# wojciech-graj/C-Raytracer

Measured on AMD Instinct MI355X. Metric: Mrays/s (primary+secondary) at 1920×1080×64spp; 1/2/4/8 GPU, higher is better.
Workload: dtype f32

## Files before the change

c-raytracer_amd/csrc/rtx_ctx.cpp:

```cpp
#include <hip/hip_runtime.h>

#include <stdarg.h>
#include <stdio.h>
#include <string.h>

#include <algorithm>
#include <vector>

#include "rtx.h"
#include "rtx_device.h"
#include "rtx_kat.h"
#include "rtx_internal.h"

static thread_local char g_err[512] = "";

int rtx_fail(int code, const char *fmt, ...)
{
	va_list ap;
	va_start(ap, fmt);
	vsnprintf(g_err, sizeof(g_err), fmt, ap);
	va_end(ap);
	return code;
}

// ... 183 lines not shown
			return fail(RTX_ERR_ARG, "shadow point masks %lld is not 0 or 1", (long long)value);
		c->opt_point = (int)value;
		return RTX_OK;
	case RTX_OPT_SHADOW_DARK:
		if (value < 0 || value > 1)
			return fail(RTX_ERR_ARG, "shadow dark samples %lld is not 0 or 1", (long long)value);
		c->opt_dark = (int)value;
		return RTX_OK;
	case RTX_OPT_SHADOW_ORDER:
		if (value < 0 || value > 1)
			return fail(RTX_ERR_ARG, "shadow sample order %lld is not 0 or 1", (long long)value);
		c->opt_order = (int)value;
		return RTX_OK;
	case RTX_OPT_SHADOW_SPEC:
		if (value < 0 || value > 1)
			return fail(RTX_ERR_ARG, "shadow specular shortcut %lld is not 0 or 1", (long long)value);
		c->opt_spec = (int)value;
		return RTX_OK;
	case RTX_OPT_SHADOW_PREMASK:
		if (value < 0 || value > 1)
			return fail(RTX_ERR_ARG, "shadow pre-mask %lld is not 0 or 1", (long long)value);
		c->opt_premask = (int)value;
		return RTX_OK;
	}
	return fail(RTX_ERR_ARG, "unknown option %d", option);
}

extern "C" int rtx_read_wide_tree(rtx_ctx *c, void *entries, uint32_t capacity, uint32_t *count, float frame[6])
{
	if (!c || !count)
		return fail(RTX_ERR_ARG, "null argument");
	if (!c->have_scene)
		return fail(RTX_ERR_STATE, "rtx_read_wide_tree before rtx_upload_scene");
	const DScene &S = c->scene;
	*count = S.w8 ? S.num_w8 : 0u;
	if (frame) {
		memcpy(frame, S.w8qo, 12);
		memcpy(frame + 3, S.w8qs, 12);
	}
	if (entries && S.w8 && capacity) {
		HIP_TRY(hipSetDevice(c->device));
		HIP_TRY(hipMemcpy(entries, S.w8, (size_t)std::min(capacity, S.num_w8) * sizeof(DW8), hipMemcpyDeviceToHost));
	}
	return RTX_OK;
}

// ... 76 lines not shown
```

c-raytracer_amd/csrc/rtx_internal.h:

```cpp
#ifndef RTX_INTERNAL_H
#define RTX_INTERNAL_H

#include <hip/hip_runtime.h>

#include <algorithm>
#include <chrono>
#include <cstdio>
#include <cstring>
#include <vector>

#include "rtx.h"
#include "rtx_device.h"
#include "rtx_launch.h"

int rtx_fail(int code, const char *fmt, ...);
#define fail rtx_fail

#define HIP_TRY(expr)                                                                                   \
	do {                                                                                            \
		hipError_t e_ = (expr);                                                                 \
		if (e_ != hipSuccess)                                                                   \
			return fail(RTX_ERR_HIP, "%s failed: %s", #expr, hipGetErrorString(e_));        \
	} while (0)

// ... 57 lines not shown
	const int rc = upload(d.p, v, stream);
	if (!rc)
		d.bytes = std::max<size_t>(v.size(), 1) * sizeof(T);
	return rc;
}

#if RTX_MEASURE
struct PhaseClock {
	std::chrono::steady_clock::time_point t = std::chrono::steady_clock::now();
	void mark(const char *what, hipStream_t st)
	{
		(void)hipStreamSynchronize(st);
		const auto n = std::chrono::steady_clock::now();
		fprintf(stderr, "[rtx upload] %-24s %8.2f ms\n", what, std::chrono::duration<double, std::milli>(n - t).count());
		t = n;
	}
};
#define PHASE(clk, what, st) clk.mark(what, st)
#else
struct PhaseClock {};
#define PHASE(clk, what, st) ((void)clk)
#endif

struct SpKey {
	uint32_t v[21] = {};
	uint32_t set = 0;
	bool operator==(const SpKey &o) const { return set && o.set && std::equal(v, v + 21, o.v); }
};

struct RTX_HIDDEN CtxHandles {
	hipStream_t stream = nullptr;
	hipEvent_t ev0 = nullptr, ev1 = nullptr;
	hipEvent_t ev[5] = { nullptr, nullptr, nullptr, nullptr, nullptr };
	CtxHandles() = default;
	CtxHandles(const CtxHandles &) = delete;
	CtxHandles &operator=(const CtxHandles &) = delete;
	~CtxHandles()
	{
		for (hipEvent_t e : { ev[0], ev[1], ev[2], ev[3], ev[4], ev0, ev1 })
			if (e)
				(void)hipEventDestroy(e);
		if (stream)
			(void)hipStreamDestroy(stream);
	}
};

struct rtx_ctx : CtxHandles {
	RTX_HIDDEN ~rtx_ctx() = default;
	int device = 0;
	int builder = RTX_BUILD_SAH_GPU;
	int cus = 0;
	DNode *d_nodes = nullptr;
	DPlane *d_planes = nullptr;
	DMaterial *d_mats = nullptr;
	DEmitter *d_emitters = nullptr;
	DEmitter *d_lin = nullptr;
	DQNode *d_qnodes = nullptr;
	uint32_t *d_top = nullptr;
	DW8 *d_w8 = nullptr;
	DW8S *d_w8s = nullptr;
	float4 *d_cull = nullptr;
	float4 *d_lsph = nullptr;
	DScene scene{};
	bool have_scene = false;
	DevBuf<DTask> d_tasks;
	DevBuf<uint32_t> d_ostk;
	DevBuf<uint32_t> d_w8spill;
	DevBuf<float4> d_staging;
	DevBuf<float4> d_sp;
	DevBuf<float4> d_contrib;
	DevBuf<uint32_t> d_ordbuf;
	DevBuf<uint32_t> d_pmask;
	DevBuf<uint2> d_tile_rec;
	double sp_tile_seen = 0.0;
	SpKey sp_tile_key{};
	DevBuf<uint32_t> d_sortbuf;
	DevBuf<void> d_sorttmp;
	DevBuf<int> d_post_rad;
	DevBuf<float4> d_post_pv;
	DevBuf<unsigned> d_post_scratch;
	float bound_lo[3] = { 0, 0, 0 }, bound_hi[3] = { 0, 0, 0 };
	uint32_t total_lights = 0;
	DevBuf<unsigned long long> d_ctr;
	DevBuf<float> d_rgb, d_z;
	rtx_stats stats{};
	rtx_point_stats pstats{};
	rtx_dark_stats dstats{};
	rtx_order_stats ostats{};
// ... 19 lines not shown
	DevBuf<double> d_ad_vs;
	DevBuf<uint32_t> d_ad_tiles;
	DevBuf<float> d_ad_var;
	DevBuf<uint32_t> d_ad_passes;
	rtx_adaptive_stats ad_stats{};
	int opt_walk = RTX_WALK_AUTO;
	uint32_t opt_leaf = 1;
	bool opt_spsort = true;
	uint32_t opt_slot = 0;
	uint32_t opt_grab = 4096;
	uint32_t opt_lstk = RTX_W8_STACK;
	int opt_trace_walk = RTX_WALK_AUTO;
	int opt_frame = RTX_FRAME_AUTO;
	uint32_t opt_chunk = 0;
	uint32_t opt_sp_tile = 0;
	uint32_t opt_rays_grab = 0;
	uint32_t opt_rays_queues = 0;
	int opt_cull = 1;
	int opt_point = 1;
	int opt_dark = 1;
	int opt_spec = 1;
	int opt_order = 1;
	int opt_premask = 1;
	uint32_t mem_share = 1;
};

struct QFrame {
	float qo[3], qs[3];
};

struct HostScene {
	int builder = RTX_BUILD_SAH_HOST;
	int device = 0;
	bool recs_on_device = false;
	std::vector<DNode> recs;
	uint32_t nnodes = 0, nb = 0, root_ref = RTX_EMPTY_REF, depth = 0;
	std::vector<DQNode> qnodes;
	QFrame qf{};
	std::vector<uint32_t> qtop;
	uint32_t ntop = 0;
	std::vector<DW8> w8;
	std::vector<uint32_t> w8leaf;
	uint32_t w8depth = 0;
	QFrame w8f{};
	bool w8noemit = false;
	bool w8_on_device = false;
// ... 110 lines not shown
```

c-raytracer_amd/csrc/rtx_launch.h:

```cpp
#ifndef RTX_LAUNCH_H
#define RTX_LAUNCH_H

#include <hip/hip_runtime.h>

#include "rtx.h"

struct DNode;
struct DPrim;
struct DW8;
struct DW8S;
struct DMaterial;
struct DScene;
struct DFrame;
struct DParams;
struct DTask;

#define RTX_HIDDEN __attribute__((visibility("hidden")))

extern "C" {

hipError_t rtx_lbvh_build(uint32_t n, const float *d_lo, const float *d_hi, const DPrim *d_prims_in, const float blo[3],
			  const float bhi[3], uint32_t max_leaf, DNode **recs_out, uint32_t *nnodes_out, uint32_t *root_out,
			  uint32_t *depth_out, hipStream_t st);
hipError_t rtx_ploc_build(uint32_t n, const float *d_lo, const float *d_hi, const DPrim *d_prims_in, const float blo[3],
			  const float bhi[3], uint32_t max_leaf, DNode **recs_out, uint32_t *nnodes_out, uint32_t *root_out,
			  uint32_t *depth_out, uint32_t *rounds_out, hipStream_t st);
hipError_t rtx_sah_build(uint32_t n, const float *d_lo, const float *d_hi, const DPrim *d_prims_in, uint32_t max_leaf,
			 uint32_t bins, uint32_t max_depth, float c_trav, float c_isect, DNode **recs_out, uint32_t *nnodes_out,
			 uint32_t *root_out, uint32_t *depth_out, uint32_t *levels_out, hipStream_t st);
hipError_t rtx_launch_find_prims(const DPrim *prims, uint32_t n, const uint32_t *objs, uint32_t nobj, uint32_t *out,
				 hipStream_t stream);
RTX_HIDDEN hipError_t rtx_load_build(void);

hipError_t rtx_launch_w8_scalar(uint32_t n, const DW8 *w8, const uint32_t *leafmap, DW8S *w8s, hipStream_t st);
hipError_t rtx_w8_collapse_device(const DNode *recs, uint32_t nnodes, uint32_t nb, const uint32_t *skip_obj,
				  uint32_t num_objects, DW8 **w8_out, DW8S **w8s_out, uint32_t **leafmap_out,
				  uint32_t *entries_out, uint32_t *scalar_entries_out, uint32_t *depth_out, uint32_t *wide_out,
				  uint32_t *top_out, float qo[3], float qs[3], hipStream_t st);
RTX_HIDDEN hipError_t rtx_load_wide8_dev(void);

size_t rtx_trace_lds_bytes(uint32_t stack_size);
hipError_t rtx_trace_occupancy(uint32_t stack_size, int *blocks_per_cu);
hipError_t rtx_launch_trace(const DScene *S, const DFrame *F, const DParams *P, float *rgb, float *z, DTask *tasks,
			    uint32_t task_cap, float4 *staging, uint32_t staging_cap, float4 *sp_out, uint32_t sp_cap,
			    uint2 *tile_rec, uint32_t tile_begin, uint32_t tile_end, unsigned long long *ctr, uint32_t waves,
			    int count, const uint32_t *tile_list, hipStream_t stream);
hipError_t rtx_launch_accum(const DFrame *F, const DParams *P, const uint2 *tile_rec, const float4 *contrib,
			    uint32_t tile_begin, uint32_t ntiles, float *rgb, const uint32_t *tile_list, hipStream_t stream);
size_t rtx_rays_lds_bytes(uint32_t stack_size);
hipError_t rtx_rays_occupancy(uint32_t stack_size, int *blocks_per_cu);
hipError_t rtx_launch_rays(const DScene *S, const float4 *rays, float4 *hits, const uint32_t *perm, uint32_t n,
			   uint32_t queues, uint32_t grab, unsigned long long *ctr, uint32_t waves, int count, int any,
			   hipStream_t stream);
hipError_t rtx_launch_frame_rays(const DFrame *F, float4 *rays, hipStream_t stream);
hipError_t rtx_launch_kat(int kind, uint32_t n, const float *in, float *out, int u32mode, hipStream_t stream);
RTX_HIDDEN hipError_t rtx_load_trace(void);

hipError_t rtx_launch_w8_fill(const DPrim *prims, const DMaterial *mats, const uint32_t *leafmap, uint32_t n, DW8 *out,
			      hipStream_t stream);
hipError_t rtx_launch_kat_shadow(int kind, uint32_t n, const float *in, float *out, hipStream_t stream);
hipError_t rtx_shadow_grid_lanes(uint32_t cus, uint32_t *lanes);
hipError_t rtx_launch_shadow(const DScene *S, const DParams *P, const float4 *sp, const uint32_t *perm, uint32_t n_sp,
			     uint32_t per_wave, uint32_t slot_b, float4 *contrib, unsigned long long *ctr, int count,
			     uint32_t cus, hipStream_t stream, uint32_t *pmask, int *premasked);
hipError_t rtx_launch_shadow_rays(const DScene *S, const float4 *rays, float4 *res, uint32_t n, unsigned long long *ctr,
				  int slots, int count, uint32_t cus, hipStream_t stream);
RTX_HIDDEN hipError_t rtx_load_shadow(void);

hipError_t rtx_spsort_temp_bytes(uint32_t n, size_t *bytes);
// ... 60 lines not shown
```

c-raytracer_amd/csrc/rtx_render.cpp:

```cpp
#include <hip/hip_runtime.h>

#include <string.h>

#include <algorithm>

#include "rtx.h"
#include "rtx_device.h"
#include "rtx_internal.h"
#include "rtx_tiles.h"

int rtx_render_common(rtx_ctx *c, const rtx_frame *fr, const rtx_params *p, float *d_rgb, float *d_z,
			 hipStream_t stream, const uint32_t *d_tiles, uint32_t n_tiles)
{
	if (!c->have_scene)
		return fail(RTX_ERR_STATE, "rtx_render before rtx_upload_scene");
	if (!fr || !p)
		return fail(RTX_ERR_ARG, "null frame/params");
	if (!fr->width || !fr->height)
		return fail(RTX_ERR_ARG, "empty frame %ux%u", fr->width, fr->height);
	if (!p->tile_stride || p->tile_offset >= p->tile_stride)
		return fail(RTX_ERR_ARG, "bad tile sharding %u/%u", p->tile_offset, p->tile_stride);
	if (d_tiles && (p->tile_offset != 0 || p->tile_stride != 1))
		return fail(RTX_ERR_ARG, "a tile list takes no tile sharding: %u/%u is not 0/1", p->tile_offset, p->tile_stride);
	const DFrame F = rtx_dframe(fr);
// ... 40 lines not shown
	sp_key.v[6] = F.width;
	sp_key.v[7] = F.height;
	memcpy(&sp_key.v[8], &P.min_intensity_sqr, 4);
	memcpy(&sp_key.v[9], F.corner, 12);
	memcpy(&sp_key.v[12], F.step_x, 12);
	memcpy(&sp_key.v[15], F.step_y, 12);
	memcpy(&sp_key.v[18], F.origin, 12);
	sp_key.set = 1;
	if (c->sp_tile_key == sp_key && c->sp_tile_seen > 0.0)
		avg_tile = std::min<uint64_t>(avg_tile, (uint64_t)(c->sp_tile_seen * 1.25) + 64);
	if (c->opt_sp_tile)
		avg_tile = c->opt_sp_tile;
	size_t free_b = 0, total_b = 0;
	HIP_TRY(hipMemGetInfo(&free_b, &total_b));
	const uint64_t budget = std::min<uint64_t>(96ull << 30, free_b / 3) / std::max<uint32_t>(c->mem_share, 1u);
	uint32_t chunk_cap = (uint32_t)std::max<uint64_t>(1, std::min<uint64_t>(P.ntiles, budget / (avg_tile * 128)));
	if (c->opt_chunk)
		chunk_cap = std::min(chunk_cap, c->opt_chunk);
	uint32_t chunk_tiles = chunk_cap;

	HIP_TRY(c->d_tasks.grow((size_t)waves * task_cap * sizeof(DTask)));
	HIP_TRY(rtx_ensure_ostk(c, waves));
	c->scene.trace_w8 = (c->scene.w8 && c->opt_trace_walk != RTX_WALK_BVH2) ? 1u : 0u;
	c->stats.trace_walk = c->scene.trace_w8 ? RTX_WALK_W8 : RTX_WALK_BVH2;
	HIP_TRY(rtx_ensure_w8spill(c, c->scene));

	HIP_TRY(hipEventRecord(c->ev0, stream));
	double t_trace = 0, t_sort = 0, t_shadow = 0, t_accum = 0;
	uint64_t shade_points = 0, premask_points = 0;
	uint32_t chunks = 0;
	unsigned long long tot[RTX_C_N] = {};
	uint32_t slot_b = 1;
	while (slot_b < 64 && slot_b < c->total_lights)
		slot_b <<= 1;
	{
		const uint32_t n = std::max<uint32_t>(c->total_lights, 1);
		const uint32_t used = slot_b * ((n + slot_b - 1) / slot_b);
		if (n > 4 && (double)n / used < 0.9)
			slot_b = 4;
	}
	if (c->opt_slot)
		slot_b = c->opt_slot;
	const uint32_t slots_per_point = (std::max<uint32_t>(c->total_lights, 1) + slot_b - 1) / slot_b;
	const uint32_t grab = c->opt_grab;
	const uint32_t per_wave = std::max<uint32_t>(1, std::min<uint32_t>(64, grab / (slot_b * slots_per_point)));
	const bool spsort = c->opt_spsort;
	bool overflowed = false;
	for (uint32_t begin = 0; begin < P.ntiles;) {
		const uint32_t end = std::min<uint32_t>(P.ntiles, begin + chunk_tiles);
		const uint64_t sp_cap64 = std::min<uint64_t>((uint64_t)(end - begin) * avg_tile + staging_cap, 0xFFFFFFF0ull);
		const uint32_t sp_cap = (uint32_t)sp_cap64;
		HIP_TRY(c->d_staging.grow((size_t)waves * staging_cap * 6 * sizeof(float4)));
		HIP_TRY(c->d_sp.grow((size_t)sp_cap * 6 * sizeof(float4)));
		HIP_TRY(c->d_contrib.grow((size_t)sp_cap * sizeof(float4)));
		if (c->opt_premask)
			HIP_TRY(c->d_pmask.grow((size_t)sp_cap * sizeof(uint32_t)));
		HIP_TRY(c->d_tile_rec.grow((size_t)(end - begin) * sizeof(uint2)));
		HIP_TRY(hipMemsetAsync(c->d_ctr, 0, sizeof(unsigned long long) * RTX_C_N, stream));
		HIP_TRY(hipEventRecord(c->ev[0], stream));
		HIP_TRY(rtx_launch_trace(&c->scene, &F, &P, d_rgb, d_z, c->d_tasks, task_cap, c->d_staging,
					 (uint32_t)staging_cap, c->d_sp, sp_cap, c->d_tile_rec, begin, end, c->d_ctr,
					 std::min<uint32_t>(waves, end - begin), p->count_traversal, d_tiles, stream));
		HIP_TRY(hipEventRecord(c->ev[1], stream));
		unsigned long long head[RTX_C_N];
		HIP_TRY(hipMemcpyAsync(head, c->d_ctr, sizeof(head), hipMemcpyDeviceToHost, stream));
		HIP_TRY(hipStreamSynchronize(stream));
		if (head[RTX_C_TASKOVERFLOW])
			return fail(RTX_ERR_STATE, "reflection/refraction task stack overflow (%u entries per wave)", task_cap);
		if (head[RTX_C_OVERFLOW]) {
			if (staging_cap >= (1ull << 26))
				return fail(RTX_ERR_STATE, "shade-point staging overflow (%llu shade points per tile)",
					    (unsigned long long)staging_cap);
			staging_cap *= 2;
			continue;
		}
		if (head[RTX_C_SPOVERFLOW]) {
			if (end - begin == 1)
				return fail(RTX_ERR_STATE, "shade-point array overflow on a single tile");
			chunk_tiles = std::max<uint32_t>(1, (end - begin) / 2);
			overflowed = true;
			continue;
		}
		const uint32_t n_sp = (uint32_t)head[RTX_C_SPCOUNT];
		shade_points += n_sp;
		const uint32_t *perm = nullptr;
// ... 236 lines not shown
```

c-raytracer_amd/csrc/rtx_trace.hip:

```cpp
#include <hip/hip_runtime.h>
#include <float.h>
#include <stdlib.h>

#include "rtx_kat.h"
#include "rtx_wave.h"
#include "rtx_w8.h"
#include "rtx_launch.h"

struct TraceCount {
	uint32_t nodes, tris, sph, pln, far;
};

template <bool COUNT, bool ANY = false, bool LIM = false>
__device__ void trace_closest_bvh2(const DScene &S, uint32_t *stk, bool act, f3 o, f3 d, uint32_t inside, float &t_out,
				   uint32_t &hid_out, TraceCount &tc)
{
	float tbest = LIM ? t_out : FLT_MAX;
	uint32_t hid = RTX_NONE;
	if (act && isnan3(d))
		act = false;
	if (act && inside != RTX_NONE) {
		float t;
		bool h;
		if (inside & RTX_PLANE_BIT) {
// ... 111 lines not shown
					if (sp == 0)
						break;
					ref = pop();
				}
			}
		}
	}
	t_out = tbest;
	hid_out = hid;
}

#ifndef RTX_TRACE_SCALAR
#define RTX_TRACE_SCALAR 1
#endif
#ifndef RTX_TRACE_NEAR
#define RTX_TRACE_NEAR 1
#endif
#ifndef RTX_TRACE_CULL
#define RTX_TRACE_CULL 0
#endif
#ifndef RTX_TRACE_EMPTYCOUNT
#define RTX_TRACE_EMPTYCOUNT 0
#endif
template <bool COUNT, int OCT, bool FAR, bool ANY = false>
__device__ __forceinline__ void closest_walk8(const DScene &S, lds_u32 *stk, uint32_t *ostk, size_t ostride, f3 o, f3 d,
					      f3 ob, f3 inv, float t0_, bool far_, float &tbest, uint32_t &hid,
					      TraceCount &tc)
{
	const float t0 = FAR ? t0_ : 0.f;
	const bool far = FAR && far_;
	uint32_t sp = 0;
	auto push = [&](uint32_t v) {
		if (sp < RTX_TRACE_LSTK)
			stk[sp * WAVE + lane_id()] = v;
		else
			ostk[(sp - RTX_TRACE_LSTK) * ostride + lane_id()] = v;
		sp++;
	};
	auto pop = [&]() -> uint32_t {
		sp--;
		return sp < RTX_TRACE_LSTK ? stk[sp * WAVE + lane_id()] : ostk[(sp - RTX_TRACE_LSTK) * ostride + lane_id()];
	};
	constexpr uint32_t K = (OCT == 8 || !RTX_W8_ORDER) ? 0u : (~(uint32_t)OCT & 7u);
	const f3 qs = ld3(S.w8qs), qo = ld3(S.w8qo);
	const f3 invq = mk3(inv.x / qs.x, inv.y / qs.y, inv.z / qs.z);
	const f3 oq = mk3((ob.x - qo.x) * qs.x, (ob.y - qo.y) * qs.y, (ob.z - qo.z) * qs.z);
	const f3 oi = mul3v(oq, invq);
	uint32_t node = 0, grp = 0;
	float gt = -INFINITY;
	constexpr bool T = RTX_TRACE_NEAR || RTX_TRACE_CULL;
	while (node != RTX_NONE) {
		W8Visit v;
		uint32_t nearp = 8;
		float tin = INFINITY;
		const uint32_t un = uni(node);
		if (RTX_TRACE_SCALAR && !ballot(node != un)) {
			if (T) {
				const W8VisitT r = w8_visit_st<OCT, K>(S.w8s + (size_t)un, invq, oi, tbest - t0);
				v = r.v;
				nearp = r.near;
				tin = r.tin;
			} else {
				v = w8_visit_s<OCT, K>(S.w8s + (size_t)un, invq, oi, tbest - t0);
			}
		} else {
			uint32_t w[16];
			const DW8 *N = S.w8 + (size_t)node;
#pragma unroll
			for (int k = 0; k < 4; k++) {
				const uint4 x = ldg4u((const uint32_t *)N + 4 * k);
				w[4 * k] = x.x;
// ... 45 lines not shown
			im &= ~(1u << p0);
			if (im) {
				if (grp)
					push(grp);
				grp = (v.base << 8) | im;
				gt = tin;
			}
		} else {
			if (RTX_TRACE_CULL && grp && gt > tbest) {
				grp = sp ? pop() : 0u;
				gt = -INFINITY;
			}
			if (grp) {
				node = (grp >> 8) + (__builtin_ctz(grp) ^ K);
				grp &= grp - 1;
				if (!(grp & 0xFFu)) {
					grp = sp ? pop() : 0u;
					gt = -INFINITY;
				}
			} else {
				node = RTX_NONE;
			}
		}
	}
}

template <bool COUNT, bool ANY = false, bool LIM = false>
__device__ void trace_closest_w8(const DScene &S, uint32_t *stk, bool act, f3 o, f3 d, uint32_t inside, float &t_out,
				 uint32_t &hid_out, TraceCount &tc)
{
	float tbest = LIM ? t_out : FLT_MAX;
	uint32_t hid = RTX_NONE;
	if (act && isnan3(d))
		act = false;
	if (act && inside != RTX_NONE) {
		float t;
		bool h;
		if (inside & RTX_PLANE_BIT) {
			const DPlane &pl = S.planes[inside & ~RTX_PLANE_BIT];
			h = hit_plane(ld3(pl.n), pl.d, o, d, pl.eps, t);
		} else {
			const DPrim &pr = S.prims[inside];
			if ((__float_as_uint(pr.c[3]) >> 24) == RTX_SPHERE)
				h = hit_sphere(mk3(pr.a[0], pr.a[1], pr.a[2]), pr.b[0], o, d, pr.a[3], t);
			else
				h = hit_triangle(mk3(pr.a[0], pr.a[1], pr.a[2]), mk3(pr.b[0], pr.b[1], pr.b[2]),
						 mk3(pr.c[0], pr.c[1], pr.c[2]), o, d, pr.a[3], t);
		}
		if (h) {
			tbest = t;
			hid = inside;
			act = false;
		}
// ... 47 lines not shown
				}
			}
		}
		lds_u32 *ls = (lds_u32 *)stk;
		uint32_t *ostk = S.ostk + (size_t)blockIdx.x * WAVE;
		const size_t ostride = (size_t)gridDim.x * WAVE;
		const uint32_t oct = ((~__float_as_uint(inv.x)) >> 31) | (((~__float_as_uint(inv.y)) >> 31) << 1) |
				     (((~__float_as_uint(inv.z)) >> 31) << 2);
		const uint32_t lead = readlane(oct, (uint32_t)__ffsll((long long)live) - 1);
		const uint32_t sel = ballot(act & (oct != lead)) ? 8u : lead;
		const bool anyfar = ballot(far) != 0;
		if (act && anyfar) {
			closest_walk8<COUNT, 8, true, ANY>(S, ls, ostk, ostride, o, d, ob, inv, t0, far, tbest, hid, tc);
		} else if (act) {
			switch (sel) {
#define RTX_CWALK(K)                                                                           \
	case K:                                                                                    \
		closest_walk8<COUNT, K, false, ANY>(S, ls, ostk, ostride, o, d, ob, inv, t0, far, tbest, hid, tc); \
		break;
				RTX_CWALK(0) RTX_CWALK(1) RTX_CWALK(2) RTX_CWALK(3) RTX_CWALK(4) RTX_CWALK(5) RTX_CWALK(6)
				RTX_CWALK(7)
#undef RTX_CWALK
			default:
				closest_walk8<COUNT, 8, false, ANY>(S, ls, ostk, ostride, o, d, ob, inv, t0, far, tbest, hid, tc);
				break;
			}
		}
	}
	t_out = tbest;
	hid_out = hid;
}

template <bool COUNT, bool ANY = false, bool LIM = false>
__device__ __forceinline__ void trace_closest(const DScene &S, uint32_t *stk, bool act, f3 o, f3 d, uint32_t inside,
					      float &t_out, uint32_t &hid_out, TraceCount &tc)
{
	if (S.trace_w8)
		trace_closest_w8<COUNT, ANY, LIM>(S, stk, act, o, d, inside, t_out, hid_out, tc);
	else
		trace_closest_bvh2<COUNT, ANY, LIM>(S, stk, act, o, d, inside, t_out, hid_out, tc);
}

struct HitInfo {
	f3 p, n;
	float b;
	bool outside;
	uint32_t obj, mat;
	float eps;
};

__device__ __forceinline__ HitInfo hit_info(const DScene &S, uint32_t hid, f3 o, f3 d, float t)
{
	HitInfo h;
// ... 91 lines not shown
		(d) = norm3(sub3(pp, (o)));                                                  \
	} while (0)

struct TraceOut {
	float4 *staging;
	uint32_t cap;
	uint32_t n;
	bool overflow;
};

__device__ __forceinline__ void emit_sp(TraceOut &T, bool has, const ShadePt &s)
{
	const u64 m = ballot(has);
	if (!m)
		return;
	const uint32_t pos = T.n + mbcnt(m);
	if (has && pos < T.cap)
		spr_store(T.staging + (size_t)pos * SPREC, s);
	T.n += popc64(m);
	if (T.n > T.cap)
		T.overflow = true;
}

template <bool COUNT>
__device__ __forceinline__ void gi_batch(const DScene &S, const DParams &P, uint32_t total_lights, uint32_t *stk,
					 float *gp_tab, uint32_t *off, uint32_t ngi_mine, f3 &acc, TraceOut &T,
					 TraceCount &tc, u64 &n_closest)
{
	uint32_t total;
	const uint32_t ex = wave_excl_scan(ngi_mine, &total);
	if (total == 0)
		return;
	lds_sync();
	off[lane_id()] = ex;
	if (lane_id() == 0)
		off[WAVE] = total;
	lds_sync();
	for (uint32_t base = 0; base < total; base += WAVE) {
		const uint32_t idx = base + lane_id();
		const bool act = idx < total;
		const uint32_t h = act ? owner_of(off, idx) : 0u;
		const GiParent par = gp_load(gp_tab, h);
		const uint32_t s = idx - off[h];
		const uint64_t pkey = key_of(par.key_lo, par.key_hi);
		float u1, u2;
		draw(P, pkey, RTX_STREAM_GI, s, u1, u2);
		const f3 dir = gi_direction(par.n, par.eps, u1, u2);
		const f3 kr = mul3s(par.w, par.delta * dot3(par.n, dir));
		const uint64_t ckey = rtx_key_child(pkey, RTX_CHILD_GI0 + s);
		float t;
		uint32_t hid;
		trace_closest<COUNT>(S, stk, act, par.p, dir, RTX_NONE, t, hid, tc);
		n_closest += popc64(ballot(act));
		const bool hit = act && hid != RTX_NONE;
		ShadePt cs = ShadePt();
		f3 cc = mk3(0.f, 0.f, 0.f);
		bool has = false;
		if (hit) {
			const HitInfo hi = hit_info(S, hid, par.p, dir, t);
			const DMaterial &m = S.mats[hi.mat];
			const f3 w = mul3s(kr, att_factor(P, t));
			cc = mul3v(w, ld3(m.ke));
			cs.nl = hi.outside ? lights_for(S, total_lights, hi.obj) : 0u;
			has = cs.nl != 0;
			cs.p = hi.p;
			cs.n = hi.n;
			cs.d = dir;
			cs.w = w;
			cs.mat = hi.mat;
			cs.obj = hi.obj | (has ? sp_far(S.tf, hi.p) : 0u);
			cs.slot = par.slot;
			cs.tex = has ? texture_color(m, hi.p, P.u32conv) : mk3(0.f, 0.f, 0.f);
			cs.key_lo = (uint32_t)ckey;
			cs.key_hi = (uint32_t)(ckey >> 32);
		}
		route_add(acc, hit, par.slot, cc);
		emit_sp(T, has, cs);
		lds_sync();
	}
}

template <bool LIST> struct TileList {};
template <> struct TileList<true> {
	const uint32_t *__restrict__ p;
};

template <bool COUNT, bool LIST>
#ifndef RTX_TRACE_OCC
#define RTX_TRACE_OCC 6
#endif
__global__ __launch_bounds__(WAVE, RTX_TRACE_OCC) void k_trace(DScene S, DFrame F, DParams P, float *__restrict__ rgb,
						float *__restrict__ zbuf, DTask *__restrict__ tasks, uint32_t task_cap,
						float4 *__restrict__ staging, uint32_t staging_cap,
						float4 *__restrict__ sp_out, uint32_t sp_cap, uint2 *__restrict__ tile_rec,
						uint32_t tile_begin, uint32_t tile_end, unsigned long long *__restrict__ ctr,
						TileList<LIST> tile_list)
{
	extern __shared__ __attribute__((aligned(16))) unsigned char lds_raw[];
	float *gp_tab = (float *)lds_raw;
	uint32_t *off = (uint32_t *)(lds_raw + WAVE * SPW * 4);
	uint32_t *stk = (uint32_t *)(lds_raw + WAVE * SPW * 4 + 80 * 4);

	uint32_t total_lights = 0;
	for (uint32_t e = 0; e < S.num_emitters; e++)
		total_lights += S.emitters[e].num_lights;
	u64 n_closest = 0;
	TraceCount tc = { 0, 0, 0, 0, 0 };
	DTask *my_tasks = tasks + (size_t)blockIdx.x * task_cap;
	TraceOut T;
	T.staging = staging + (size_t)blockIdx.x * staging_cap * SPREC;
	T.cap = staging_cap;
	bool overflow = false, task_overflow = false, sp_overflow = false;

	for (;;) {
		uint32_t tile = 0;
		if (lane_id() == 0)
			tile = (uint32_t)atomicAdd(&ctr[RTX_C_TILE], 1ull);
		tile = uni(__shfl(tile, 0, WAVE)) + tile_begin;
		if (tile >= tile_end)
// ... 106 lines not shown
							my_tasks[pos_r] = tk;
						}
						if (want_refr) {
							const uint64_t k2 = rtx_key_child(key, RTX_CHILD_REFRACT);
							DTask tk;
							tk.o[0] = sp.p.x; tk.o[1] = sp.p.y; tk.o[2] = sp.p.z;
							tk.d[0] = tdir.x; tk.d[1] = tdir.y; tk.d[2] = tdir.z;
							tk.kr[0] = rkt.x; tk.kr[1] = rkt.y; tk.kr[2] = rkt.z;
							tk.rb = rb - 1;
							tk.inside = hid;
							tk.key_lo = (uint32_t)k2;
							tk.key_hi = (uint32_t)(k2 >> 32);
							tk.slot = slot;
							my_tasks[pos_t] = tk;
						}
						top += nr + nt;
					}
				}
			}
			if (P.gi == RTX_GI_PATH) {
				lds_sync();
				if (hit)
					gp_store(gp_tab, lane_id(), gp);
				gi_batch<COUNT>(S, P, total_lights, stk, gp_tab, off, hit ? gp.ngi : 0u, acc, T, tc,
						n_closest);
			}
			if (top == 0)
				break;
			__builtin_amdgcn_fence(__ATOMIC_SEQ_CST, "workgroup");
			const uint32_t n = min(top, (uint32_t)WAVE);
			top -= n;
			act = lane_id() < n;
			primary = false;
			if (act) {
				const DTask tk = my_tasks[top + lane_id()];
				o = ld3(tk.o);
				d = ld3(tk.d);
				kr = ld3(tk.kr);
				rb = tk.rb;
				inside = tk.inside;
				key = key_of(tk.key_lo, tk.key_hi);
				slot = tk.slot;
			}
			__builtin_amdgcn_fence(__ATOMIC_SEQ_CST, "workgroup");
		}
		if (valid_px) {
			const size_t pix = (size_t)py * F.width + px;
			if (rgb) {
// ... 292 lines not shown
	} break;
	case RTX_KAT_REFRACT: {
		f3 dd = ld3(x), nn = ld3(x + 3);
		float b = dot3(nn, dd);
		f3 r = refract_dir(dd, nn, b, signbit(b), x[6]);
		y[0] = r.x;
		y[1] = r.y;
		y[2] = r.z;
	} break;
	}
}

extern "C" size_t rtx_trace_lds_bytes(uint32_t stack_size)
{
	size_t pad = 0;
#if RTX_MEASURE
	const char *e = getenv("RTX_TRACE_LDS_PAD");
	pad = e ? (size_t)atoi(e) : 0;
#endif
	const size_t lstk = stack_size < RTX_TRACE_LSTK ? stack_size : RTX_TRACE_LSTK;
	return (size_t)WAVE * SPW * 4 + 80 * 4 + lstk * WAVE * 4 + pad;
}

extern "C" hipError_t rtx_trace_occupancy(uint32_t stack_size, int *blocks_per_cu)
{
	return hipOccupancyMaxActiveBlocksPerMultiprocessor(blocks_per_cu, k_trace<false, false>, WAVE,
							     rtx_trace_lds_bytes(stack_size));
}

extern "C" hipError_t rtx_launch_trace(const DScene *S, const DFrame *F, const DParams *P, float *rgb, float *z,
				       DTask *tasks, uint32_t task_cap, float4 *staging, uint32_t staging_cap,
				       float4 *sp_out, uint32_t sp_cap, uint2 *tile_rec, uint32_t tile_begin,
				       uint32_t tile_end, unsigned long long *ctr, uint32_t waves, int count,
				       const uint32_t *tile_list, hipStream_t stream)
{
	const size_t lds = rtx_trace_lds_bytes(S->stack_size);
#define RTX_TRACE_LAUNCH(C, L, ...) \
	hipLaunchKernelGGL((k_trace<C, L>), dim3(waves), dim3(WAVE), lds, stream, *S, *F, *P, rgb, z, tasks, task_cap, staging, \
			   staging_cap, sp_out, sp_cap, tile_rec, tile_begin, tile_end, ctr, TileList<L>{ __VA_ARGS__ })
	if (tile_list && count)
		RTX_TRACE_LAUNCH(true, true, tile_list);
	else if (tile_list)
		RTX_TRACE_LAUNCH(false, true, tile_list);
	else if (count)
		RTX_TRACE_LAUNCH(true, false);
	else
		RTX_TRACE_LAUNCH(false, false);
#undef RTX_TRACE_LAUNCH
	return hipGetLastError();
}

extern "C" hipError_t rtx_launch_accum(const DFrame *F, const DParams *P, const uint2 *tile_rec,
				       const float4 *contrib, uint32_t tile_begin, uint32_t ntiles, float *rgb,
				       const uint32_t *tile_list, hipStream_t stream)
{
	if (!ntiles || !rgb)
		return hipSuccess;
	if (tile_list)
		hipLaunchKernelGGL(k_accum<true>, dim3(ntiles), dim3(WAVE), 0, stream, *F, *P, tile_rec, contrib, tile_begin, rgb,
				   TileList<true>{ tile_list });
	else
		hipLaunchKernelGGL(k_accum<false>, dim3(ntiles), dim3(WAVE), 0, stream, *F, *P, tile_rec, contrib, tile_begin, rgb,
// ... 55 lines not shown
```

c-raytracer_amd/rtxpy/abi.py:

```python
import ctypes as C

RTX_OK = 0
RTX_ERR_ARG, RTX_ERR_HIP, RTX_ERR_NOMEM, RTX_ERR_SCENE, RTX_ERR_NODEV, RTX_ERR_STATE, RTX_ERR_IO = (
    -1, -2, -3, -4, -5, -6, -7)

RTX_SPHERE, RTX_TRIANGLE, RTX_PLANE = 0, 1, 2
RTX_TEX_UNIFORM, RTX_TEX_CHECKERBOARD, RTX_TEX_BRICK, RTX_TEX_NOISY_PERIODIC = 0, 1, 2, 3
RTX_PHONG, RTX_BLINN = 0, 1
RTX_GI_AMBIENT, RTX_GI_PATH = 0, 1
RTX_ATT_NONE, RTX_ATT_LIN, RTX_ATT_SQR = 0, 1, 2
RTX_RNG_COUNTER, RTX_RNG_CONST, RTX_RNG_STRAT = 0, 1, 2
RTX_U32_SAT, RTX_U32_WRAP = 0, 1

F3 = C.c_float * 3


class Material(C.Structure):
    _fields_ = [("id", C.c_int32), ("ks", F3), ("ka", F3), ("kr", F3), ("kt", F3), ("ke", F3),
                ("shininess", C.c_float), ("refractive_index", C.c_float), ("texture", C.c_int32),
                ("periodic", C.c_int32), ("color", F3 * 2), ("scale", C.c_float), ("mortar_width", C.c_float),
                ("noise_feature_scale", C.c_float), ("noise_scale", C.c_float), ("frequency_scale", C.c_float),
                ("emittant", C.c_int32), ("reflective", C.c_int32), ("transparent", C.c_int32)]


# ... 63 lines not shown

class PremaskStats(C.Structure):
    _fields_ = [("premask_points", C.c_uint64)]


RTX_TRANSPORT_NONE, RTX_TRANSPORT_RCCL, RTX_TRANSPORT_LOOPBACK, RTX_TRANSPORT_RCCL_SELF = 0, 1, 2, 3


class GroupMember(C.Structure):
    _fields_ = [("device", C.c_int32), ("comm_count", C.c_int32), ("comm_rank", C.c_int32), ("comm_device", C.c_int32),
                ("can_access_peer0", C.c_uint32), ("peer0_can_access", C.c_uint32), ("peer_enabled", C.c_uint32),
                ("transport", C.c_uint32), ("pci_bus_id", C.c_char * 32)]


RTX_BUILD_SAH_HOST, RTX_BUILD_LBVH_GPU, RTX_BUILD_PLOC_GPU, RTX_BUILD_SAH_GPU = 0, 1, 2, 3
RTX_WALK_AUTO, RTX_WALK_BVH2, RTX_WALK_W8, RTX_WALK_LINEAR = -1, 0, 2, 3
WALK_NAMES = {RTX_WALK_BVH2: "bvh2", RTX_WALK_W8: "w8", RTX_WALK_LINEAR: "linear"}
RTX_SHADOW_LINEAR_MAX = 8
RTX_FRAME_AUTO, RTX_FRAME_WORLD = 0, 1
RTX_OPT_SHADOW_WALK, RTX_OPT_BVH_LEAF, RTX_OPT_SPSORT, RTX_OPT_SHADOW_SLOT, RTX_OPT_SHADOW_GRAB, \
    RTX_OPT_SHADOW_LDS_STACK, RTX_OPT_TRACE_WALK, RTX_OPT_TREE_FRAME, RTX_OPT_CHUNK_TILES, \
    RTX_OPT_SP_PER_TILE, RTX_OPT_SHADOW_CULL, RTX_OPT_RAYS_GRAB, RTX_OPT_RAYS_QUEUES, \
    RTX_OPT_SHADOW_POINT, RTX_OPT_SHADOW_DARK, RTX_OPT_SHADOW_PREMASK, RTX_OPT_SHADOW_ORDER, \
    RTX_OPT_SHADOW_SPEC = 1, 2, 3, 4, 5, 6, 7, 8, 9, 10, 11, 12, 13, 14, 15, 16, 17, 18
RTX_DOF_NONE, RTX_DOF_SCALE_BIAS, RTX_DOF_CAMERA = 0, 1, 2
RTX_FALLOFF_QUAD, RTX_FALLOFF_LIN, RTX_FALLOFF_INV_QUAD = 0, 1, 2


class Post(C.Structure):
    _fields_ = [("brighten", C.c_int32), ("brighten_factor", C.c_float), ("dof", C.c_int32),
                ("dof_scale", C.c_float), ("dof_bias", C.c_float), ("aperture", C.c_float),
                ("focal_length", C.c_float), ("plane_in_focus", C.c_float), ("mist", C.c_int32),
                ("mist_start", C.c_float), ("mist_depth", C.c_float), ("mist_falloff", C.c_int32),
                ("mist_color", F3)]


RTX_RAYS_ANY_HIT, RTX_RAYS_REORDER, RTX_RAYS_COUNT = 1, 2, 4
RTX_RAYS_MAX = 0x7FFFFFFF


class Ray(C.Structure):
    _fields_ = [("origin", F3), ("tmax", C.c_float), ("dir", F3), ("pad_", C.c_uint32)]


class Hit(C.Structure):
    _fields_ = [("t", C.c_float), ("object", C.c_int32), ("material", C.c_int32), ("outside", C.c_uint32),
                ("n", F3), ("pad_", C.c_uint32)]
# ... 352 lines not shown
```

include/rtx.h:

```cpp
#ifndef RTX_H
#define RTX_H

#include <stddef.h>
#include <stdint.h>

#ifdef __cplusplus
extern "C" {
#endif

#define RTX_ABI_VERSION 1

enum rtx_status {
	RTX_OK = 0,
	RTX_ERR_ARG = -1,
	RTX_ERR_HIP = -2,
	RTX_ERR_NOMEM = -3,
	RTX_ERR_SCENE = -4,
	RTX_ERR_NODEV = -5,
	RTX_ERR_STATE = -6,
	RTX_ERR_IO = -7,
};

enum rtx_object_type { RTX_SPHERE = 0, RTX_TRIANGLE = 1, RTX_PLANE = 2 };

// ... 192 lines not shown
enum {
	RTX_FRAME_AUTO = 0,
	RTX_FRAME_WORLD = 1
};
enum rtx_option {
	RTX_OPT_SHADOW_WALK = 1,
	RTX_OPT_BVH_LEAF = 2,
	RTX_OPT_SPSORT = 3,
	RTX_OPT_SHADOW_SLOT = 4,
	RTX_OPT_SHADOW_GRAB = 5,
	RTX_OPT_SHADOW_LDS_STACK = 6,
	RTX_OPT_TRACE_WALK = 7,
	RTX_OPT_TREE_FRAME = 8,
	RTX_OPT_CHUNK_TILES = 9,
	RTX_OPT_SP_PER_TILE = 10,
	RTX_OPT_SHADOW_CULL = 11,
	RTX_OPT_RAYS_GRAB = 12,
	RTX_OPT_RAYS_QUEUES = 13,
	RTX_OPT_SHADOW_POINT = 14,
	RTX_OPT_SHADOW_DARK = 15,
	RTX_OPT_SHADOW_PREMASK = 16,
	RTX_OPT_SHADOW_ORDER = 17,
	RTX_OPT_SHADOW_SPEC = 18,
};
int rtx_set_option(rtx_ctx *ctx, int option, int64_t value);
int rtx_tree_frame(const rtx_scene_desc *scene, int *rotated, float rot[9], float center[3], double *cost_ratio);
void rtx_close(rtx_ctx *ctx);
const char *rtx_last_error(void);
int rtx_read_wide_tree(rtx_ctx *ctx, void *entries, uint32_t capacity, uint32_t *count, float frame[6]);
int rtx_read_bvh2(rtx_ctx *ctx, void *records, uint32_t record_capacity, uint32_t *num_nodes, uint32_t *num_prims,
		  uint32_t *root_ref, void *qnodes, uint32_t qnode_capacity, uint32_t *num_qnodes, float qframe[6]);

typedef struct rtx_ray {
	float origin[3];
	float tmax;
	float dir[3];
	uint32_t pad_;
} rtx_ray;
typedef struct rtx_hit {
	float t;
	int32_t object;
	int32_t material;
	uint32_t outside;
	float n[3];
	uint32_t pad_;
} rtx_hit;
// ... 222 lines not shown
```

Measured before the change: 63350.

## Compact GI ray traversal via root-step queue and packed resume pass

Splits GI closest-hit tracing into a first pass that expands only the wide-BVH root for each ray, a queue in global scratch that records rays still needing traversal, and a resume pass that walks the queued rays packed densely across lanes, followed by a separate shading pass. The aim is to cut SIMD divergence from rays that terminate early while others walk deep. In exchange it adds global-memory traffic for per-ray results and queue entries, extra fences and recomputation of GI ray directions, and a per-block scratch buffer. It is enabled by default for path-traced GI with the wide tree.

```diff
diff --git a/c-raytracer_amd/csrc/rtx_ctx.cpp b/c-raytracer_amd/csrc/rtx_ctx.cpp
--- a/c-raytracer_amd/csrc/rtx_ctx.cpp
+++ b/c-raytracer_amd/csrc/rtx_ctx.cpp
@@ -229,6 +229,11 @@
 			return fail(RTX_ERR_ARG, "shadow pre-mask %lld is not 0 or 1", (long long)value);
 		c->opt_premask = (int)value;
 		return RTX_OK;
+	case RTX_OPT_TRACE_PACK:
+		if (value != 0 && value != 1 && value != 512 && value != 1024 && value != 2048 && value != 4096)
+			return fail(RTX_ERR_ARG, "trace pack %lld is not 0, 1, 512, 1024, 2048 or 4096", (long long)value);
+		c->opt_trace_pack = (uint32_t)value;
+		return RTX_OK;
 	}
 	return fail(RTX_ERR_ARG, "unknown option %d", option);
 }
diff --git a/c-raytracer_amd/csrc/rtx_internal.h b/c-raytracer_amd/csrc/rtx_internal.h
--- a/c-raytracer_amd/csrc/rtx_internal.h
+++ b/c-raytracer_amd/csrc/rtx_internal.h
@@ -103,6 +103,10 @@
 #define PHASE(clk, what, st) ((void)clk)
 #endif
 
+#ifndef RTX_TRACE_PACK_SEG
+#define RTX_TRACE_PACK_SEG 4096u
+#endif
+
 struct SpKey {
 	uint32_t v[21] = {};
 	uint32_t set = 0;
@@ -145,6 +149,7 @@
 	DScene scene{};
 	bool have_scene = false;
 	DevBuf<DTask> d_tasks;
+	DevBuf<void> d_pack;
 	DevBuf<uint32_t> d_ostk;
 	DevBuf<uint32_t> d_w8spill;
 	DevBuf<float4> d_staging;
@@ -210,6 +215,7 @@
 	int opt_spec = 1;
 	int opt_order = 1;
 	int opt_premask = 1;
+	uint32_t opt_trace_pack = 1;
 	uint32_t mem_share = 1;
 };
 
diff --git a/c-raytracer_amd/csrc/rtx_launch.h b/c-raytracer_amd/csrc/rtx_launch.h
--- a/c-raytracer_amd/csrc/rtx_launch.h
+++ b/c-raytracer_amd/csrc/rtx_launch.h
@@ -39,12 +39,13 @@
 				  uint32_t *top_out, float qo[3], float qs[3], hipStream_t st);
 RTX_HIDDEN hipError_t rtx_load_wide8_dev(void);
 
+size_t rtx_trace_pack_bytes(uint32_t pack_seg);
 size_t rtx_trace_lds_bytes(uint32_t stack_size);
 hipError_t rtx_trace_occupancy(uint32_t stack_size, int *blocks_per_cu);
 hipError_t rtx_launch_trace(const DScene *S, const DFrame *F, const DParams *P, float *rgb, float *z, DTask *tasks,
 			    uint32_t task_cap, float4 *staging, uint32_t staging_cap, float4 *sp_out, uint32_t sp_cap,
 			    uint2 *tile_rec, uint32_t tile_begin, uint32_t tile_end, unsigned long long *ctr, uint32_t waves,
-			    int count, const uint32_t *tile_list, hipStream_t stream);
+			    int count, const uint32_t *tile_list, void *pack, uint32_t pack_seg, hipStream_t stream);
 hipError_t rtx_launch_accum(const DFrame *F, const DParams *P, const uint2 *tile_rec, const float4 *contrib,
 			    uint32_t tile_begin, uint32_t ntiles, float *rgb, const uint32_t *tile_list, hipStream_t stream);
 size_t rtx_rays_lds_bytes(uint32_t stack_size);
diff --git a/c-raytracer_amd/csrc/rtx_render.cpp b/c-raytracer_amd/csrc/rtx_render.cpp
--- a/c-raytracer_amd/csrc/rtx_render.cpp
+++ b/c-raytracer_amd/csrc/rtx_render.cpp
@@ -86,6 +86,10 @@
 	HIP_TRY(c->d_tasks.grow((size_t)waves * task_cap * sizeof(DTask)));
 	HIP_TRY(rtx_ensure_ostk(c, waves));
 	c->scene.trace_w8 = (c->scene.w8 && c->opt_trace_walk != RTX_WALK_BVH2) ? 1u : 0u;
+	const uint32_t pack_seg = c->opt_trace_pack == 1 ? RTX_TRACE_PACK_SEG : c->opt_trace_pack;
+	const bool pack = pack_seg && c->scene.trace_w8 && P.gi == RTX_GI_PATH;
+	if (pack)
+		HIP_TRY(c->d_pack.grow((size_t)waves * rtx_trace_pack_bytes(pack_seg)));
 	c->stats.trace_walk = c->scene.trace_w8 ? RTX_WALK_W8 : RTX_WALK_BVH2;
 	HIP_TRY(rtx_ensure_w8spill(c, c->scene));
 
@@ -124,7 +128,8 @@
 		HIP_TRY(hipEventRecord(c->ev[0], stream));
 		HIP_TRY(rtx_launch_trace(&c->scene, &F, &P, d_rgb, d_z, c->d_tasks, task_cap, c->d_staging,
 					 (uint32_t)staging_cap, c->d_sp, sp_cap, c->d_tile_rec, begin, end, c->d_ctr,
-					 std::min<uint32_t>(waves, end - begin), p->count_traversal, d_tiles, stream));
+					 std::min<uint32_t>(waves, end - begin), p->count_traversal, d_tiles,
+					 pack ? (void *)c->d_pack : nullptr, pack_seg, stream));
 		HIP_TRY(hipEventRecord(c->ev[1], stream));
 		unsigned long long head[RTX_C_N];
 		HIP_TRY(hipMemcpyAsync(head, c->d_ctr, sizeof(head), hipMemcpyDeviceToHost, stream));
diff --git a/c-raytracer_amd/csrc/rtx_trace.hip b/c-raytracer_amd/csrc/rtx_trace.hip
--- a/c-raytracer_amd/csrc/rtx_trace.hip
+++ b/c-raytracer_amd/csrc/rtx_trace.hip
@@ -157,10 +157,10 @@
 #ifndef RTX_TRACE_EMPTYCOUNT
 #define RTX_TRACE_EMPTYCOUNT 0
 #endif
-template <bool COUNT, int OCT, bool FAR, bool ANY = false>
+template <bool COUNT, int OCT, bool FAR, bool ANY = false, bool ONE = false>
 __device__ __forceinline__ void closest_walk8(const DScene &S, lds_u32 *stk, uint32_t *ostk, size_t ostride, f3 o, f3 d,
 					      f3 ob, f3 inv, float t0_, bool far_, float &tbest, uint32_t &hid,
-					      TraceCount &tc)
+					      TraceCount &tc, uint32_t node = 0, uint32_t grp = 0, uint2 *left = nullptr)
 {
 	const float t0 = FAR ? t0_ : 0.f;
 	const bool far = FAR && far_;
@@ -181,7 +181,6 @@
 	const f3 invq = mk3(inv.x / qs.x, inv.y / qs.y, inv.z / qs.z);
 	const f3 oq = mk3((ob.x - qo.x) * qs.x, (ob.y - qo.y) * qs.y, (ob.z - qo.z) * qs.z);
 	const f3 oi = mul3v(oq, invq);
-	uint32_t node = 0, grp = 0;
 	float gt = -INFINITY;
 	constexpr bool T = RTX_TRACE_NEAR || RTX_TRACE_CULL;
 	while (node != RTX_NONE) {
@@ -273,13 +272,19 @@
 				node = RTX_NONE;
 			}
 		}
-	}
-}
-
-template <bool COUNT, bool ANY = false, bool LIM = false>
+		if (ONE)
+			break;
+	}
+	if (ONE)
+		*left = make_uint2(node, grp);
+}
+
+template <bool COUNT, bool ANY = false, bool LIM = false, bool ROOT = false>
 __device__ void trace_closest_w8(const DScene &S, uint32_t *stk, bool act, f3 o, f3 d, uint32_t inside, float &t_out,
-				 uint32_t &hid_out, TraceCount &tc)
-{
+				 uint32_t &hid_out, TraceCount &tc, uint2 *left = nullptr)
+{
+	if (ROOT)
+		*left = make_uint2(RTX_NONE, 0u);
 	float tbest = LIM ? t_out : FLT_MAX;
 	uint32_t hid = RTX_NONE;
 	if (act && isnan3(d))
@@ -373,13 +378,29 @@
 				RTX_CWALK(7)
 #undef RTX_CWALK
 			default:
-				closest_walk8<COUNT, 8, false, ANY>(S, ls, ostk, ostride, o, d, ob, inv, t0, far, tbest, hid, tc);
+				if constexpr (ROOT)
+					closest_walk8<COUNT, 8, false, ANY, true>(S, ls, ostk, ostride, o, d, ob, inv, t0, far, tbest,
+										  hid, tc, 0u, 0u, left);
+				else
+					closest_walk8<COUNT, 8, false, ANY>(S, ls, ostk, ostride, o, d, ob, inv, t0, far, tbest, hid, tc);
 				break;
 			}
 		}
 	}
 	t_out = tbest;
 	hid_out = hid;
+}
+
+template <bool COUNT>
+__device__ __forceinline__ void resume_closest_w8(const DScene &S, uint32_t *stk, bool act, f3 o, f3 d, uint2 at,
+						  float &tbest, uint32_t &hid, TraceCount &tc)
+{
+	const bool rot = S.tf.rotated != 0;
+	const f3 ob = rot ? tf_point(S.tf.r, S.tf.c, o) : o;
+	const f3 inv = safe_inv_fast(rot ? tf_dir(S.tf.r, d) : d);
+	if (act)
+		closest_walk8<COUNT, 8, false>(S, (lds_u32 *)stk, S.ostk + (size_t)blockIdx.x * WAVE, (size_t)gridDim.x * WAVE, o,
+					       d, ob, inv, 0.f, false, tbest, hid, tc, at.x, at.y);
 }
 
 template <bool COUNT, bool ANY = false, bool LIM = false>
@@ -517,6 +538,55 @@
 		T.overflow = true;
 }
 
+__device__ __forceinline__ void gi_shade(const DScene &S, const DParams &P, uint32_t total_lights, bool act,
+					 const GiParent &par, f3 dir, f3 kr, uint64_t ckey, float t, uint32_t hid, f3 &acc,
+					 TraceOut &T)
+{
+	const bool hit = act && hid != RTX_NONE;
+	ShadePt cs = ShadePt();
+	f3 cc = mk3(0.f, 0.f, 0.f);
+	bool has = false;
+	if (hit) {
+		const HitInfo hi = hit_info(S, hid, par.p, dir, t);
+		const DMaterial &m = S.mats[hi.mat];
+		const f3 w = mul3s(kr, att_factor(P, t));
+		cc = mul3v(w, ld3(m.ke));
+		cs.nl = hi.outside ? lights_for(S, total_lights, hi.obj) : 0u;
+		has = cs.nl != 0;
+		cs.p = hi.p;
+		cs.n = hi.n;
+		cs.d = dir;
+		cs.w = w;
+		cs.mat = hi.mat;
+		cs.obj = hi.obj | (has ? sp_far(S.tf, hi.p) : 0u);
+		cs.slot = par.slot;
+		cs.tex = has ? texture_color(m, hi.p, P.u32conv) : mk3(0.f, 0.f, 0.f);
+		cs.key_lo = (uint32_t)ckey;
+		cs.key_hi = (uint32_t)(ckey >> 32);
+	}
+	route_add(acc, hit, par.slot, cc);
+	emit_sp(T, has, cs);
+}
+
+struct GiRay {
+	GiParent par;
+	uint32_t s;
+	uint64_t pkey;
+	f3 dir;
+};
+__device__ __forceinline__ GiRay gi_ray(const DParams &P, const float *gp_tab, const uint32_t *off, bool act, uint32_t idx)
+{
+	GiRay r;
+	const uint32_t h = act ? owner_of(off, idx) : 0u;
+	r.par = gp_load(gp_tab, h);
+	r.s = idx - off[h];
+	r.pkey = key_of(r.par.key_lo, r.par.key_hi);
+	float u1, u2;
+	draw(P, r.pkey, RTX_STREAM_GI, r.s, u1, u2);
+	r.dir = gi_direction(r.par.n, r.par.eps, u1, u2);
+	return r;
+}
+
 template <bool COUNT>
 __device__ __forceinline__ void gi_batch(const DScene &S, const DParams &P, uint32_t total_lights, uint32_t *stk,
 					 float *gp_tab, uint32_t *off, uint32_t ngi_mine, f3 &acc, TraceOut &T,
@@ -534,45 +604,94 @@
 	for (uint32_t base = 0; base < total; base += WAVE) {
 		const uint32_t idx = base + lane_id();
 		const bool act = idx < total;
-		const uint32_t h = act ? owner_of(off, idx) : 0u;
-		const GiParent par = gp_load(gp_tab, h);
-		const uint32_t s = idx - off[h];
-		const uint64_t pkey = key_of(par.key_lo, par.key_hi);
-		float u1, u2;
-		draw(P, pkey, RTX_STREAM_GI, s, u1, u2);
-		const f3 dir = gi_direction(par.n, par.eps, u1, u2);
-		const f3 kr = mul3s(par.w, par.delta * dot3(par.n, dir));
-		const uint64_t ckey = rtx_key_child(pkey, RTX_CHILD_GI0 + s);
+		const GiRay r = gi_ray(P, gp_tab, off, act, idx);
+		const f3 kr = mul3s(r.par.w, r.par.delta * dot3(r.par.n, r.dir));
+		const uint64_t ckey = rtx_key_child(r.pkey, RTX_CHILD_GI0 + r.s);
 		float t;
 		uint32_t hid;
-		trace_closest<COUNT>(S, stk, act, par.p, dir, RTX_NONE, t, hid, tc);
+		trace_closest<COUNT>(S, stk, act, r.par.p, r.dir, RTX_NONE, t, hid, tc);
 		n_closest += popc64(ballot(act));
-		const bool hit = act && hid != RTX_NONE;
-		ShadePt cs = ShadePt();
-		f3 cc = mk3(0.f, 0.f, 0.f);
-		bool has = false;
-		if (hit) {
-			const HitInfo hi = hit_info(S, hid, par.p, dir, t);
-			const DMaterial &m = S.mats[hi.mat];
-			const f3 w = mul3s(kr, att_factor(P, t));
-			cc = mul3v(w, ld3(m.ke));
-			cs.nl = hi.outside ? lights_for(S, total_lights, hi.obj) : 0u;
-			has = cs.nl != 0;
-			cs.p = hi.p;
-			cs.n = hi.n;
-			cs.d = dir;
-			cs.w = w;
-			cs.mat = hi.mat;
-			cs.obj = hi.obj | (has ? sp_far(S.tf, hi.p) : 0u);
-			cs.slot = par.slot;
-			cs.tex = has ? texture_color(m, hi.p, P.u32conv) : mk3(0.f, 0.f, 0.f);
-			cs.key_lo = (uint32_t)ckey;
-			cs.key_hi = (uint32_t)(ckey >> 32);
-		}
-		route_add(acc, hit, par.slot, cc);
-		emit_sp(T, has, cs);
+		gi_shade(S, P, total_lights, act, r.par, r.dir, kr, ckey, t, hid, acc, T);
 		lds_sync();
 	}
+}
+
+template <bool PACK> struct TracePack {};
+template <> struct TracePack<true> {
+	unsigned char *__restrict__ buf;
+	uint32_t seg;
+};
+#define RTX_PACK_BYTES 24
+
+template <bool COUNT>
+__device__ __forceinline__ void gi_batch_packed(const DScene &S, const DParams &P, uint32_t total_lights, uint32_t *stk,
+						float *gp_tab, uint32_t *off, uint32_t ngi_mine, f3 &acc, TraceOut &T,
+						TraceCount &tc, u64 &n_closest, const TracePack<true> &pack)
+{
+	static_assert(!RTX_TRACE_CULL, "the queue does not carry the kept group's entry distance");
+	uint32_t total;
+	const uint32_t ex = wave_excl_scan(ngi_mine, &total);
+	if (total == 0)
+		return;
+	lds_sync();
+	off[lane_id()] = ex;
+	if (lane_id() == 0)
+		off[WAVE] = total;
+	lds_sync();
+	uint2 *res = (uint2 *)(pack.buf + (size_t)blockIdx.x * pack.seg * RTX_PACK_BYTES);
+	uint4 *queue = (uint4 *)(res + pack.seg);
+	for (uint32_t s0 = 0; s0 < total; s0 += pack.seg) {
+		const uint32_t s1 = min(total, s0 + pack.seg);
+		uint32_t nq = 0;
+		for (uint32_t base = s0; base < s1; base += WAVE) {
+			const uint32_t idx = base + lane_id();
+			const bool act = idx < total;
+			const GiRay r = gi_ray(P, gp_tab, off, act, idx);
+			float t;
+			uint32_t hid;
+			uint2 left;
+			trace_closest_w8<COUNT, false, false, true>(S, stk, act, r.par.p, r.dir, RTX_NONE, t, hid, tc, &left);
+			n_closest += popc64(ballot(act));
+			if (act)
+				res[idx - s0] = make_uint2(__float_as_uint(t), hid);
+			const bool more = left.x != RTX_NONE;
+			const u64 m = ballot(more);
+			if (more)
+				queue[nq + mbcnt(m)] = make_uint4(idx, left.x, left.y, 0u);
+			nq += popc64(m);
+			lds_sync();
+		}
+		__builtin_amdgcn_fence(__ATOMIC_SEQ_CST, "workgroup");
+		for (uint32_t qb = 0; qb < nq; qb += WAVE) {
+			const bool act = qb + lane_id() < nq;
+			uint4 e = make_uint4(s0, RTX_NONE, 0u, 0u);
+			if (act)
+				e = queue[qb + lane_id()];
+			const GiRay r = gi_ray(P, gp_tab, off, act, e.x);
+			uint2 th = make_uint2(0u, RTX_NONE);
+			if (act)
+				th = res[e.x - s0];
+			float t = __uint_as_float(th.x);
+			resume_closest_w8<COUNT>(S, stk, act, r.par.p, r.dir, make_uint2(e.y, e.z), t, th.y, tc);
+			if (act)
+				res[e.x - s0] = make_uint2(__float_as_uint(t), th.y);
+			lds_sync();
+		}
+		__builtin_amdgcn_fence(__ATOMIC_SEQ_CST, "workgroup");
+		for (uint32_t base = s0; base < s1; base += WAVE) {
+			const uint32_t idx = base + lane_id();
+			const bool act = idx < total;
+			const GiRay r = gi_ray(P, gp_tab, off, act, idx);
+			uint2 th = make_uint2(0u, RTX_NONE);
+			if (act)
+				th = res[idx - s0];
+			const f3 kr = mul3s(r.par.w, r.par.delta * dot3(r.par.n, r.dir));
+			const uint64_t ckey = rtx_key_child(r.pkey, RTX_CHILD_GI0 + r.s);
+			gi_shade(S, P, total_lights, act, r.par, r.dir, kr, ckey, __uint_as_float(th.x), th.y, acc, T);
+		}
+		__builtin_amdgcn_fence(__ATOMIC_SEQ_CST, "workgroup");
+	}
+	lds_sync();
 }
 
 template <bool LIST> struct TileList {};
@@ -580,7 +699,7 @@
 	const uint32_t *__restrict__ p;
 };
 
-template <bool COUNT, bool LIST>
+template <bool COUNT, bool LIST, bool PACK>
 #ifndef RTX_TRACE_OCC
 #define RTX_TRACE_OCC 6
 #endif
@@ -589,7 +708,7 @@
 						float4 *__restrict__ staging, uint32_t staging_cap,
 						float4 *__restrict__ sp_out, uint32_t sp_cap, uint2 *__restrict__ tile_rec,
 						uint32_t tile_begin, uint32_t tile_end, unsigned long long *__restrict__ ctr,
-						TileList<LIST> tile_list)
+						TileList<LIST> tile_list, TracePack<PACK> pack)
 {
 	extern __shared__ __attribute__((aligned(16))) unsigned char lds_raw[];
 	float *gp_tab = (float *)lds_raw;
@@ -742,8 +861,12 @@
 				lds_sync();
 				if (hit)
 					gp_store(gp_tab, lane_id(), gp);
-				gi_batch<COUNT>(S, P, total_lights, stk, gp_tab, off, hit ? gp.ngi : 0u, acc, T, tc,
-						n_closest);
+				if constexpr (PACK)
+					gi_batch_packed<COUNT>(S, P, total_lights, stk, gp_tab, off, hit ? gp.ngi : 0u, acc, T,
+							       tc, n_closest, pack);
+				else
+					gi_batch<COUNT>(S, P, total_lights, stk, gp_tab, off, hit ? gp.ngi : 0u, acc, T, tc,
+							n_closest);
 			}
 			if (top == 0)
 				break;
@@ -1082,9 +1205,14 @@
 	return (size_t)WAVE * SPW * 4 + 80 * 4 + lstk * WAVE * 4 + pad;
 }
 
+extern "C" size_t rtx_trace_pack_bytes(uint32_t pack_seg)
+{
+	return (size_t)pack_seg * RTX_PACK_BYTES;
+}
+
 extern "C" hipError_t rtx_trace_occupancy(uint32_t stack_size, int *blocks_per_cu)
 {
-	return hipOccupancyMaxActiveBlocksPerMultiprocessor(blocks_per_cu, k_trace<false, false>, WAVE,
+	return hipOccupancyMaxActiveBlocksPerMultiprocessor(blocks_per_cu, k_trace<false, false, false>, WAVE,
 							     rtx_trace_lds_bytes(stack_size));
 }
 
@@ -1092,12 +1220,22 @@
 				       DTask *tasks, uint32_t task_cap, float4 *staging, uint32_t staging_cap,
 				       float4 *sp_out, uint32_t sp_cap, uint2 *tile_rec, uint32_t tile_begin,
 				       uint32_t tile_end, unsigned long long *ctr, uint32_t waves, int count,
-				       const uint32_t *tile_list, hipStream_t stream)
+				       const uint32_t *tile_list, void *pack, uint32_t pack_seg, hipStream_t stream)
 {
 	const size_t lds = rtx_trace_lds_bytes(S->stack_size);
-#define RTX_TRACE_LAUNCH(C, L, ...) \
-	hipLaunchKernelGGL((k_trace<C, L>), dim3(waves), dim3(WAVE), lds, stream, *S, *F, *P, rgb, z, tasks, task_cap, staging, \
-			   staging_cap, sp_out, sp_cap, tile_rec, tile_begin, tile_end, ctr, TileList<L>{ __VA_ARGS__ })
+	if (pack && (!S->trace_w8 || !pack_seg || pack_seg % WAVE))
+		return hipErrorInvalidValue;
+#define RTX_TRACE_LAUNCH(C, L, ...)                                                                                            \
+	do {                                                                                                                    \
+		if (pack)                                                                                                       \
+			hipLaunchKernelGGL((k_trace<C, L, true>), dim3(waves), dim3(WAVE), lds, stream, *S, *F, *P, rgb, z, tasks,  \
+					   task_cap, staging, staging_cap, sp_out, sp_cap, tile_rec, tile_begin, tile_end, ctr,     \
+					   TileList<L>{ __VA_ARGS__ }, TracePack<true>{ (unsigned char *)pack, pack_seg });        \
+		else                                                                                                            \
+			hipLaunchKernelGGL((k_trace<C, L, false>), dim3(waves), dim3(WAVE), lds, stream, *S, *F, *P, rgb, z, tasks, \
+					   task_cap, staging, staging_cap, sp_out, sp_cap, tile_rec, tile_begin, tile_end, ctr,     \
+					   TileList<L>{ __VA_ARGS__ }, TracePack<false>{});                                        \
+	} while (0)
 	if (tile_list && count)
 		RTX_TRACE_LAUNCH(true, true, tile_list);
 	else if (tile_list)
diff --git a/c-raytracer_amd/rtxpy/abi.py b/c-raytracer_amd/rtxpy/abi.py
--- a/c-raytracer_amd/rtxpy/abi.py
+++ b/c-raytracer_amd/rtxpy/abi.py
@@ -109,7 +109,7 @@
     RTX_OPT_SHADOW_LDS_STACK, RTX_OPT_TRACE_WALK, RTX_OPT_TREE_FRAME, RTX_OPT_CHUNK_TILES, \
     RTX_OPT_SP_PER_TILE, RTX_OPT_SHADOW_CULL, RTX_OPT_RAYS_GRAB, RTX_OPT_RAYS_QUEUES, \
     RTX_OPT_SHADOW_POINT, RTX_OPT_SHADOW_DARK, RTX_OPT_SHADOW_PREMASK, RTX_OPT_SHADOW_ORDER, \
-    RTX_OPT_SHADOW_SPEC = 1, 2, 3, 4, 5, 6, 7, 8, 9, 10, 11, 12, 13, 14, 15, 16, 17, 18
+    RTX_OPT_SHADOW_SPEC, RTX_OPT_TRACE_PACK = 1, 2, 3, 4, 5, 6, 7, 8, 9, 10, 11, 12, 13, 14, 15, 16, 17, 18, 19
 RTX_DOF_NONE, RTX_DOF_SCALE_BIAS, RTX_DOF_CAMERA = 0, 1, 2
 RTX_FALLOFF_QUAD, RTX_FALLOFF_LIN, RTX_FALLOFF_INV_QUAD = 0, 1, 2
 
diff --git a/include/rtx.h b/include/rtx.h
--- a/include/rtx.h
+++ b/include/rtx.h
@@ -238,6 +238,7 @@
 	RTX_OPT_SHADOW_PREMASK = 16,
 	RTX_OPT_SHADOW_ORDER = 17,
 	RTX_OPT_SHADOW_SPEC = 18,
+	RTX_OPT_TRACE_PACK = 19,
 };
 int rtx_set_option(rtx_ctx *ctx, int option, int64_t value);
 int rtx_tree_frame(const rtx_scene_desc *scene, int *rotated, float rot[9], float center[3], double *cost_ratio);
```

New measurement: 64130 (median of 6 runs). 1.01x the previous value.
